# tatsy/opengl-raytracer

Measured on AMD Instinct MI355X. Metric: Mrays/s at 1920x1080, 8 bounces, higher is better.
Workload: dtype f32

## Files before the change

### opengl-raytracer_amd/csrc/glrtx.hip

```cpp
#include "glrtx.h"

#include <hip/hip_runtime.h>

#include <algorithm>
#include <cmath>
#include <cstdarg>
#include <cstdio>
#include <cstdlib>
#include <cstring>
#include <new>
#include <limits>
#include <string>
#include <vector>

#include "glrt_host.h"
#include "pt_kernel.hip.h"
#include "lbvh.hip.h"
#include "sahl.hip.h"
#include "refit.hip.h"
#include "query.hip.h"
#include "features.hip.h"
#include "denoise.hip.h"
#include "variance.hip.h"
#include "reproject.hip.h"
// ... 893 lines not shown
    P.ring = ring;
    P.inv_gamma = 1.0f / gamma;
    P.flip = flip ? 1 : 0;
    P.full = full;
    P.seq = P.acq = 0;
    P.timed = false;
    if (c->width > 0) {
        int rc = ensure(c, P.dev, present_image_bytes(c) * (size_t)ring);
        for (auto &im : P.img) {
            if (rc != GLRTX_OK || full) break;
            const hipError_t e = hipHostMalloc((void **)&im.host, std::max<size_t>(present_image_bytes(c), 64), hipHostMallocPortable);
            if (e != hipSuccess) rc = fail(c, GLRTX_ENOMEM, "glrtx_present_enable: pinned host memory: %s", hipGetErrorString(e));
            else im.host_bytes = std::max<size_t>(present_image_bytes(c), 64);
        }
        if (rc != GLRTX_OK) { (void)present_stop(c); return rc; }
    }
    return GLRTX_OK;
}

bool present_held(const glrtx_ctx *c) {
    for (const auto &im : c->pres.img)
        if (im.state == glrtx_ctx::Present::Image::HELD) return true;
    return false;
}

int wgwf_fetch(const glrtx_ctx *c, bool vine) {
    int fetch = vine ? 0 : ((size_t)c->n_fork + (size_t)c->st.n_tri >= (size_t)kPairFetchMinRecords ? 1 : 0);
    if (const char *v = std::getenv("GLRTX_PAIR_FETCH")) fetch = vine ? 0 : std::max(0, std::min(2, std::atoi(v)));
    return fetch;
}

int wgwf_lds_base(const glrtx_ctx *c) {
    return c->sc.lds_head_f4 * (int)sizeof(float4) + 2 * c->sc.stack_entries * kBlockThreads * (int)sizeof(int) + kWgCtlWords * (int)sizeof(unsigned) +
           2 * (int)sizeof(float4) + kCamFloatsPadded * (int)sizeof(float) + kLdsSeeds * (int)sizeof(float2) + kWgPathsMax / 8;
}

bool wgwf_compact(const glrtx_ctx *c, bool vine, int fetch) {
    const int lds_compact = wgwf_lds_base(c) + c->sc.n_crank * (int)sizeof(uint2);
    bool compact = !vine && fetch == 0 && c->sc.n_crank > 0 && (size_t)lds_compact * GLRTX_WGWF_WAVES <= (size_t)160 * 1024;
    if (const char *v = std::getenv("GLRTX_COMPACT_NODES")) compact = std::atoi(v) != 0 && !vine && fetch == 0 && c->sc.n_crank > 0 && lds_compact <= 160 * 1024;
    return compact;
}

int launch_wgwf(glrtx_ctx *c, const KernelArgs &a_in, const glrtx_params *p, const float *seeds_xy, int n_frames) {
    KernelArgs a = a_in;
    const int tiles8_x = (c->width + 7) / 8, tiles8_y = (c->owned_rows + 7) / 8;
    const size_t total = (size_t)tiles8_x * tiles8_y * 64;
    if (total * 2 >= (size_t)INT32_MAX) return fail(c, GLRTX_EINVAL, "image too large for the wgwf variant");
    const size_t plane_bytes = (size_t)a.pitch_f4 * (size_t)c->owned_rows * sizeof(float4);
    const size_t frame_bytes = (size_t)std::max(p->n_samples, 1) * plane_bytes;
    int rc;
    const bool busy = c->last_render_done && hipEventQuery(c->last_render_done) == hipErrorNotReady;
    (void)hipGetLastError();
    const bool burst = c->last_was_render && busy && same_camera(c->last_p, *p);
    const bool adapt = c->adapt_launch;
    const bool vol = c->ext_flags != 0;
    const bool moments = c->moments_launch;
    bool fed = !adapt && !moments && c->feed_ok && std::getenv("GLRTX_NO_FEED") == nullptr && c->pipeline && c->stream == c->own_stream && p->n_samples >= 1 && seeds_xy != nullptr && (n_frames > 1 || burst);
    int fed_cap = fed ? std::min(frames_cap(c, p, (int)kFedSlots), kFeedMaxFrames) : 0;
    if (const char *v = std::getenv("GLRTX_FEED_CAP")) fed_cap = std::max(1, std::min(fed_cap, std::atoi(v)));
    if (fed && n_frames > fed_cap) fed = false;
    bool piped = fed || (!adapt && !moments && n_frames == 1 && c->pipeline && p->n_samples >= 1 && (size_t)p->n_samples * plane_bytes <= ((size_t)1 << 30));
    const size_t ids = total * (size_t)(fed ? fed_cap : n_frames);
    if (ids + 1 >= (size_t)UINT32_MAX)
        return fail(c, GLRTX_EINVAL, "glrtx_render_frames: %d frames of %zu pixels exceed the 32-bit ray id space", n_frames, total);

    using Kernel = void (*)(const KernelArgs, const WfArgs, unsigned *, float4 *, const int *, const unsigned *, const VolArgs);
// ... 128 lines not shown
    w.tiles8_x = tiles8_x;
    w.refill_min = kRefillMin;
    if (const char *v = std::getenv("GLRTX_REFILL_MIN")) w.refill_min = std::max(1, std::min(64, std::atoi(v)));
    w.n_frames = fed ? std::max(fed_cap, 2) : n_frames;
    w.tiles_per_frame = (int)(total >> 6);
    const size_t plane_f4 = (size_t)a.pitch_f4 * (size_t)c->owned_rows;
    const int n_planes = n_frames * p->n_samples;
    if (fed) {
        FeedHost *fh = slot->feed_h;
        for (int i = 0; i < n_frames; i++) fh->seeds[i] = make_float2(seeds_xy[2 * i], seeds_xy[2 * i + 1]);
        __atomic_store_n(&fh->frames_pub, (unsigned)n_frames, __ATOMIC_RELEASE);
        w.feed_host = slot->feed_h_dev;
        w.feed_dev = (FeedDev *)slot->feed_d.p;
        w.feed_plane_f4 = plane_f4;
        w.feed_margin = 64 * 4 * grid;
        if (const char *v = std::getenv("GLRTX_FEED_MARGIN")) w.feed_margin = std::max(0, std::atoi(v));
    } else {
        if (n_frames > 1) {
            if ((rc = ensure(c, c->wfSeeds, (size_t)n_frames * sizeof(float2)))) return rc;
            HIP_TRY(c, hipMemcpyAsync(c->wfSeeds.p, seeds_xy, (size_t)n_frames * sizeof(float2), hipMemcpyHostToDevice, c->stream));
            w.seeds = (const float2 *)c->wfSeeds.p;
            w.seeds_in_lds = n_frames <= kLdsSeeds ? 1 : 0;
        }
        if (n_frames > 1 || slot || adapt || moments) {
            if ((rc = ensure(c, planeBuf, (size_t)std::max(n_planes, 1) * plane_f4 * sizeof(float4)))) return rc;
            w.planes = (float4 *)planeBuf.p;
        }
    }
    w.block_paths = block_paths;
    w.gss_div = (slot && !fed) ? 0 : 4 * grid;
    if (const char *v = std::getenv("GLRTX_GSS_DIV")) w.gss_div = std::max(0, std::atoi(v));
    w.suspend_max = kSuspendMax;
    if (const char *v = std::getenv("GLRTX_SUSPEND_MAX")) w.suspend_max = std::max(0, std::min(64, std::atoi(v)));
    w.trip_limit = (int)std::min<long long>(INT32_MAX, 64ll * std::max(p->n_samples, 1) * (p->max_depth + 2) + 64);
    if (vol) w.trip_limit = (int)std::min<long long>(INT32_MAX, 64ll * std::max(p->n_samples, 1) * 9 * (p->max_depth + 2) + 64);
    if (const char *v = std::getenv("GLRTX_TRIP_LIMIT")) w.trip_limit = std::max(1, std::atoi(v));
    w.err = c->guard_dev;
    {
        const size_t max_id = ids - 1;
        const size_t max_sidx = (size_t)kWfSetPlanes * state_entries + (size_t)grid * block_paths - 1;
        const size_t slice_f4 = 2 * (size_t)2 * 2 * block_paths  + (2 * (size_t)block_paths * sizeof(unsigned) + 15) / 16 ;
        static_assert(kWgSuspendAt + (size_t)kSuspendF4 * kBlockThreads == kWgQueueF4, "the suspend area closes a workgroup's slice");
        bool ok = slice_f4 <= kWgSuspendAt && max_id < (size_t)WF_INVALID && 2 * max_sidx + 1 < (size_t)WF_INVALID && (size_t)grid * block_paths <= state_entries &&
                  (size_t)kWfStatePlanes * state_entries * sizeof(float4) < ((size_t)1 << 32) && (block_paths & (block_paths - 1)) == 0 && block_paths >= 256 &&
                  block_paths <= kWgPathsMax && slice_f4 <= kWgQueueF4 && queueBuf.bytes >= (size_t)grid * kWgQueueF4 * sizeof(float4) &&
                  stateBuf.bytes >= state_bytes && w.ids == state_entries && grid >= 1 && (size_t)grid <= wg_slots &&
                  p->max_depth <= kWfDepthMax && p->n_samples <= kWfSampleMax && workPtr != nullptr;
        if (vol) ok = ok && p->n_samples <= kWfVolSampleMax && c->ext_flags == GLRTX_EXT_VOLUME && c->have_volume && c->vol.density != nullptr &&
                      c->vol.temperature != nullptr && c->n_spheres == 0 && !vine && fetch == 0 && !compact;
        if (!fed && n_frames > 1) ok = ok && c->wfSeeds.bytes >= (size_t)n_frames * sizeof(float2);
        if (w.planes) ok = ok && planeBuf.bytes >= (size_t)std::max(n_planes, 1) * plane_f4 * sizeof(float4);
        if (adapt) ok = ok && !fed && !slot && w.planes && c->ad_selected && c->ad_tiles == (int)(total >> 6) && c->adList.bytes >= (total >> 6) * sizeof(int) &&
                      c->adMask.bytes >= (total >> 6) && c->adHalf.bytes >= (size_t)c->ad_pitch * c->owned_rows && c->ad_pitch == c->pitch_bytes;
        if (moments) ok = ok && !fed && !slot && w.planes && c->mmM.p && c->mm_pitch == c->pitch_bytes && c->mm_rows == c->owned_rows &&
                        c->mmM.bytes >= c->pitch_bytes * (size_t)c->owned_rows;
        if (fed) ok = ok && n_frames >= 1 && n_frames <= fed_cap && fed_cap <= kFeedMaxFrames && slot->feed_d.bytes >= sizeof(FeedDev) && w.feed_host != nullptr &&
                      slot->chunks[(n_frames - 1) / kFeedChunkFrames].p != nullptr && slot->chunk_bytes == frame_bytes;
        if (!ok) return fail(c, GLRTX_EDEVICE, "internal: wgwf launch shapes inconsistent (ids %zu, max id %zu, grid %d of %zu slots (%d per CU), block_paths %d, frames %d, fed %d)", ids, max_id,
                             grid, wg_slots, per_cu, block_paths, n_frames, (int)fed);
        (void)queue_bytes_max;
    }
    glrtx_ctx::LaunchRec *rec = nullptr;
    if ((rc = next_launch_rec(c, rec))) return rc;
    if (slot && slot->used) HIP_TRY(c, hipStreamWaitEvent(rstream, slot->acc_done, 0));
    if (ctx_state && c->state_used) HIP_TRY(c, hipStreamWaitEvent(rstream, c->state_done, 0));
    HIP_TRY(c, hipMemsetAsync(workPtr, 0, sizeof(unsigned), rstream));
// ... 2680 lines not shown
```

### opengl-raytracer_amd/csrc/pt_kernel.hip.h

```cpp
#pragma once
#include <hip/hip_runtime.h>
#include <stdint.h>

#include "trav_asm.hip.h"
#include "scan_asm.hip.h"

namespace glrtx {

constexpr int kBlockThreads = 256;
constexpr int kTile = 16;
constexpr int REF_ABSENT = INT32_MIN;
constexpr int REF_FIN = INT32_MIN;
constexpr int kMaxLdsMaterials = 256;
constexpr int kMaxLdsLights = 64;
constexpr int kTopForks = 128;

constexpr float PT_EPS = 1.0e-4f;
constexpr float PT_INFTY = 1.0e8f;
constexpr float PT_PI = 3.14159274101257324f;
constexpr float PT_2PI = 6.28318548202514648f;

struct DevScene {
    const float4 *forks;
    const float4 *nodes0;
// ... 1406 lines not shown
struct FeedDev {
    unsigned frames_known;
    unsigned pad[31];
    unsigned long long seeds[kFeedMaxFrames];
    unsigned long long chunks[kFeedChunks];
};
constexpr int kCamFloatsPadded = 36;
constexpr int kLdsSeeds = 64;
constexpr int kWfSetPlanes = 6;
struct WfArgs {
    float4 *state;
    size_t ids;
    DEV size_t plane(int k) const { size_t n = ids; asm volatile("" : "+s"(n)); return (size_t)k * n; }
    DEV float4 *A(int k, unsigned sidx) const { return reinterpret_cast<float4 *>(reinterpret_cast<char *>(state + plane(k)) + (size_t)(sidx * 16u)); }
    DEV float4 *H(unsigned sidx) const { return A(5, sidx); }
    DEV unsigned set_base(int set, int wg) const { size_t n = ids; asm volatile("" : "+s"(n)); return (unsigned)((size_t)set * kWfSetPlanes * n) + (unsigned)wg * (unsigned)block_paths; }
    int total;
    int tiles8_x;
    int refill_min;
    int block_paths;
    int gss_div;
    int suspend_max;
    int trip_limit;
    unsigned *err;
    FeedHost *feed_host;
    FeedDev *feed_dev;
    size_t feed_plane_f4;
    int feed_margin;
    const float2 *seeds;
    int seeds_in_lds;
    float4 *planes;
    int n_frames;
    int tiles_per_frame;
    DEV void split(int id, int &frame, int &pid) const {
        if (n_frames > 1) { frame = (int)((unsigned)id / (unsigned)total); pid = id - frame * total; }
        else { frame = 0; pid = id; }
    }
};
constexpr int kWfStatePlanes = 2 * kWfSetPlanes;
constexpr int kWfDepthMax = 255;
constexpr int kWfSampleMax = (1 << 20) - 1;
constexpr int kWfVolSampleMax = (1 << 16) - 1;
constexpr unsigned kWfVolShift = 24;
constexpr unsigned kWfVolPassed = 9;
constexpr unsigned WF_PENDING = 1u << 28;
constexpr unsigned WF_FINISHING = 1u << 29;
constexpr unsigned WF_RESOLVED = 1u << 30;
constexpr unsigned WF_ACCEPTED = 1u << 31;
constexpr unsigned WF_INVALID = 0xFFFFFFFFu;
constexpr int kSuspendMax = 24;
constexpr float kHitSuspended = -1.0f;
constexpr int kSuspendF4 = 4;
constexpr int kRefillMin = 16;
#ifdef GLRTX_FAULT_INJECT
constexpr unsigned kFaultPoison = 0xFFFFFFFEu;
#endif

DEV bool wf_pixel(const KernelArgs &a, const WfArgs &w, int id, int &lx, int &lrow) {
    int frame, pid;
    w.split(id, frame, pid);
    const int t = pid >> 6, k = pid & 63;
    lx = (t % w.tiles8_x) * 8 + (k & 7);
    lrow = (t / w.tiles8_x) * 8 + (k >> 3);
    return lx < a.width && lrow < a.owned_rows;
}

// ... 219 lines not shown
    }
    if (ended) {
        int lx, lrow;
        wf_pixel(a, w, (int)id, lx, lrow);
        const int gy = local_row_to_y(a, lrow);
        const float fcx = (float)lx + 0.5f, fcy = (float)gy + 0.5f;
        wf_add_sample(a, w, (int)id, lx, lrow, sample, P.Lx, P.Ly, P.Lz);
        sample++;
        push_ext = wf_start(a, w, cam, (int)id, lx, lrow, rng, fcx, fcy, P, sample);
        if (push_ext) {
            ray_o = make_float4(P.ox, P.oy, P.oz, rng.x);
            ray_d = make_float4(P.dx, P.dy, P.dz, rng.y);
            st2 = make_float4(1.f, 1.f, 1.f, __uint_as_float(sample << 8));
            st3 = make_float4(0.f, 0.f, 0.f, s3.w);
        }
    } else {
        push_sh = sh.has_shadow;
        push_ext = !sh.ended;
        const unsigned m2 = (unsigned)P.depth | (sample << 8) | (push_sh ? WF_PENDING : 0u) | (sh.ended ? WF_FINISHING : 0u);
        ray_o = make_float4(P.ox, P.oy, P.oz, rng.x);
        ray_d = make_float4(P.dx, P.dy, P.dz, rng.y);
        st2 = make_float4(P.bx, P.by, P.bz, __uint_as_float(m2));
        st3 = make_float4(sh.Lpx, sh.Lpy, sh.Lpz, s3.w);
        if (push_sh) { st4 = make_float4(sh.Lfx, sh.Lfy, sh.Lfz, 0.f); has4 = true; }
        ray_sd = make_float4(sh.sdx, sh.sdy, sh.sdz, sh.dist);
    }
}

#ifndef GLRTX_STEPS_PER_TRIP
#define GLRTX_STEPS_PER_TRIP 6
#endif
constexpr int kWgCtlWords = 32;
constexpr int kWgPathsMax = 4096;
constexpr size_t kWgSuspendAt = 8 * (size_t)kWgPathsMax + (size_t)kWgPathsMax / 2;
constexpr size_t kWgQueueF4 = kWgSuspendAt + (size_t)kSuspendF4 * kBlockThreads;
#ifndef GLRTX_PRIO_TRAVERSE
#define GLRTX_PRIO_TRAVERSE 3
#define GLRTX_PRIO_SHADE 0
#endif
#ifndef GLRTX_WGWF_WAVES
#define GLRTX_WGWF_WAVES 4
#endif

#ifdef GLRTX_PHASE_STATS
__device__ unsigned long long g_phase_cycles[8];
__device__ uint4 g_trip_log[16][64];
#define PH_STAMP(var) const unsigned long long var = __builtin_amdgcn_s_memtime()
#define PH_ADD(i, t0, t1) do { if (threadIdx.x == 0) atomicAdd(&g_phase_cycles[i], (t1) - (t0)); } while (0)
#else
#define PH_STAMP(var)
#define PH_ADD(i, t0, t1)
#endif

#ifdef GLRTX_RAY_LOG
struct RayLog { float4 *rays; uint2 *trips; unsigned long long cap_rays; unsigned cap_trips; unsigned on; };
__device__ RayLog g_ray_log;
__device__ unsigned long long g_ray_log_n;
__device__ unsigned g_ray_log_trips;
#endif

DEV int wgwf_suspend_max();

template <bool VINE, int FETCH>
DEV void wg_traverse_phase(const KernelArgs &a, const WfArgs &w, const float4 *root, int *stack, const float4 *rq, int n_rays,
                           unsigned *ray_head, unsigned *light_bits, unsigned long long &rays, float4 *suspend_area) {
    const int lane = threadIdx.x & 63;
    const uint2 *ranks = reinterpret_cast<const uint2 *>(light_bits + kWgPathsMax / 32);
    if (VINE) {
        for (;;) {
            int base = 0;
            if (lane == 0) base = (int)atomicAdd(ray_head, 64u);
            base = __builtin_amdgcn_readfirstlane(base);
            if (base >= n_rays) break;
            float4 o = make_float4(0.f, 0.f, 0.f, __uint_as_float(WF_INVALID)), d = o;
            if (base + lane < n_rays) { o = ld_stream(&rq[2 * (size_t)(base + lane)]); d = ld_stream(&rq[2 * (size_t)(base + lane) + 1]); }
            const unsigned r = __float_as_uint(o.w);
            const bool shadow = (r & 1u) != 0u;
            const Hit h = trav_scan<true>(a.sc, o.x, o.y, o.z, d.x, d.y, d.z, r != WF_INVALID, shadow ? shadow_limit(d.w, a.sc.shadow_limited) : PT_INFTY,
                                          shadow ? d.w : -__builtin_inff());
            if (r != WF_INVALID) {
                rays++;
                if (r & 1u) { if (nee_accepted(d.w, h.t, h.tri >= 0)) atomicOr(&light_bits[r >> 6], 1u << ((r >> 1) & 31u)); }
                else st_stream(w.H(r >> 1), make_float4(h.t, __int_as_float(h.tri), h.u, h.v));
            }
        }
        return;
    }
    const unsigned long long lt_mask = (1ull << lane) - 1ull;
    const float4 none = make_float4(0.f, 0.f, 0.f, __uint_as_float(WF_INVALID));
    float4 cur_o = none, cur_d = none;
    float cur_ix = 0.f, cur_iy = 0.f, cur_iz = 0.f;
    int cur_pos = 0, cur_cnt = 0;
    auto fetch = [&](float4 &o, float4 &d) -> int {
        int base = 0;
        if (lane == 0) base = (int)atomicAdd(ray_head, 64u);
        base = __builtin_amdgcn_readfirstlane(base);
        int cnt = n_rays - base;
        cnt = cnt < 0 ? 0 : (cnt > 64 ? 64 : cnt);
        if (lane < cnt) {
            o = ld_stream(&rq[2 * (size_t)(base + lane)]);
// ... 12 lines not shown
    bool active = false;
    bool unsaved = false;
    unsigned rid = 0;
    Trav T;
    T.cur = 0; T.sp = 0;
    T.h.t = PT_INFTY; T.h.tri = -1; T.h.u = 0.f; T.h.v = 0.f;
#ifdef GLRTX_STEP_TIMING
    StepTiming step_timing;
#endif
    float4 *const susp = suspend_area + (size_t)kSuspendF4 * threadIdx.x;
    {
        const float4 s3 = susp[3];
        if (s3.z != 0.0f) {
            const float4 s0 = susp[0], s1 = susp[1], s2 = susp[2];
            susp[3] = make_float4(0.f, 0.f, 0.f, 0.f);
            T.ox = s0.x; T.oy = s0.y; T.oz = s0.z;
            rid = __float_as_uint(w.H(__float_as_uint(s0.w) >> 1)->y);
#ifdef GLRTX_FAULT_INJECT
            const bool fault_dropped = rid == kFaultPoison;
#endif
            T.dx = s1.x; T.dy = s1.y; T.dz = s1.z; T.stop_d = s1.w;
            T.ix = frcp(T.dx); T.iy = frcp(T.dy); T.iz = frcp(T.dz);
            T.h.t = s2.x; T.h.tri = __float_as_int(s2.y); T.h.u = s2.z; T.h.v = s2.w;
            T.cur = __float_as_int(s3.x); T.sp = __float_as_int(s3.y);
#ifdef GLRTX_TRAV_STATS
            T.iters = 0;
#endif
            active = true;
#ifdef GLRTX_FAULT_INJECT
            if (fault_dropped) active = false;
#endif
        }
    }
    auto save_hit = [&]() {
        const unsigned id = rid >> 1;
        if (rid & 1u) {
            if (nee_accepted(T.stop_d, T.h.t, T.h.tri >= 0)) atomicOr(&light_bits[id >> 5], 1u << (id & 31u));
        } else *w.H(id) = make_float4(T.h.t, __int_as_float(T.h.tri), T.h.u, T.h.v);
        unsaved = false;
    };
#ifdef GLRTX_PHASE_STATS
    unsigned long long ph_refill = 0ull, ph_refills = 0ull, ph_step = 0ull;
#endif
    for (;;) {
        unsigned long long idle = __ballot(!active);
        if ((int)__popcll(idle) >= w.refill_min || idle == ~0ull) {
#ifdef GLRTX_PHASE_STATS
            const unsigned long long rf0 = __builtin_amdgcn_s_memtime();
#endif
            while (idle != 0ull && !exhausted) {
                if (cur_pos >= cur_cnt) {
                    cur_cnt = cur_cnt == 64 ? fetch(cur_o, cur_d) : 0;
                    cur_pos = 0;
                    if (cur_cnt == 0) { exhausted = true; break; }
                }
                const int n = __popcll(idle);
                const int avail = cur_cnt - cur_pos;
                const int take = n < avail ? n : avail;
                const int rank = __popcll(idle & lt_mask);
                const int src = (cur_pos + rank) & 63;
                const float ox = __shfl(cur_o.x, src), oy = __shfl(cur_o.y, src), oz = __shfl(cur_o.z, src);
                const unsigned new_rid = (unsigned)__shfl((int)__float_as_uint(cur_o.w), src);
                const float dx = __shfl(cur_d.x, src), dy = __shfl(cur_d.y, src), dz = __shfl(cur_d.z, src);
                const float dist_m = __shfl(cur_d.w, src);
                const float ix = __shfl(cur_ix, src), iy = __shfl(cur_iy, src), iz = __shfl(cur_iz, src);
                if (!active && rank < take) {
                    if (unsaved) save_hit();
                    rid = new_rid;
                    if (rid != WF_INVALID) {
                        rays++;
                        const bool shadow = (rid & 1u) != 0u;
                        const float dist = __builtin_fabsf(dist_m);
                        T.ox = ox; T.oy = oy; T.oz = oz; T.dx = dx; T.dy = dy; T.dz = dz; T.ix = ix; T.iy = iy; T.iz = iz;
                        T.h.t = shadow ? shadow_limit(dist, a.sc.shadow_limited) : PT_INFTY; T.h.tri = -1; T.h.u = 0.f; T.h.v = 0.f;
                        T.stop_d = shadow ? dist : -__builtin_inff();
                        T.sp = 0;
                        T.cur = (FETCH & kWgwfCompact) ? 0 : a.sc.root_ref;
#ifdef GLRTX_TRAV_STATS
                        T.iters = 0;
#endif
                        active = (__float_as_uint(dist_m) & 0x80000000u) == 0u;
                        unsaved = !active;
                    }
                }
                cur_pos += take;
                idle = __ballot(!active);
            }
#ifdef GLRTX_PHASE_STATS
            ph_refill += __builtin_amdgcn_s_memtime() - rf0; ph_refills += 1ull;
#endif
        }
        if (!__any(active)) {
            if (exhausted) break;
            continue;
        }
        if (exhausted && fetched_any) {
            const unsigned long long ma = __ballot(active);
            const int suspend_max = wgwf_suspend_max();
            if (__ballot(active && (rid & 1u) != 0u) == 0ull && (int)__popcll(ma) <= suspend_max) {
                if (active) {
                    susp[0] = make_float4(T.ox, T.oy, T.oz, __uint_as_float(rid));
                    susp[1] = make_float4(T.dx, T.dy, T.dz, T.stop_d);
                    susp[2] = make_float4(T.h.t, __int_as_float(T.h.tri), T.h.u, T.h.v);
                    susp[3] = make_float4(__int_as_float(T.cur), __int_as_float(T.sp), 1.0f, 0.f);
                    float mark = kHitSuspended, zero = 0.f;
                    asm volatile("" : "+v"(mark), "+v"(zero));
                    *w.H(rid >> 1) = make_float4(mark, zero, zero, zero);
                    active = false;
                }
                break;
            }
        }
#ifdef GLRTX_PHASE_STATS
        const unsigned long long sb0 = __builtin_amdgcn_s_memtime();
#endif
#ifdef GLRTX_TRAV_STATS
        {
            const unsigned long long ma = __ballot(active);
            if (lane == 0) {
                atomicAdd(&g_trav_trips[0], 1ull); atomicAdd(&g_trav_trips[1], (unsigned long long)__popcll(ma));
                if (exhausted) { atomicAdd(&g_trav_trips[2], 1ull); atomicAdd(&g_trav_trips[3], (unsigned long long)__popcll(ma)); }
            }
        }
#endif
        if (active) {
#if defined(GLRTX_TRAV_STATS) || defined(GLRTX_CXX_STEP)
            constexpr bool CP = (FETCH & kWgwfCompact) != 0;
            bool fin = trav_step<true, CP>(a.sc, stack, T, ranks);
#pragma unroll
            for (int k = 1; k < GLRTX_STEPS_PER_TRIP; k++)
                if (!fin) fin = trav_step<true, CP>(a.sc, stack, T, ranks);
#else
#ifdef GLRTX_STEP_TIMING
            trav_steps_asm<FETCH>(a.sc, stack, T, (unsigned)(uintptr_t)ranks, step_timing);
#else
            trav_steps_asm<FETCH>(a.sc, stack, T, (unsigned)(uintptr_t)ranks);
#endif
            const bool fin = T.cur == REF_FIN;
#endif
            if (fin) {
                active = false;
                unsaved = true;
            }
        }
#ifdef GLRTX_PHASE_STATS
        ph_step += __builtin_amdgcn_s_memtime() - sb0;
#endif
    }
    if (unsaved) save_hit();
#ifdef GLRTX_PHASE_STATS
    if (threadIdx.x == 0) { atomicAdd(&g_phase_cycles[5], ph_refill); atomicAdd(&g_phase_cycles[6], ph_refills); atomicAdd(&g_phase_cycles[7], ph_step); }
#endif
#ifdef GLRTX_STEP_TIMING
    atomicAdd(&g_step_timing[0], (unsigned long long)step_timing.n);
    atomicAdd(&g_step_timing[1], (unsigned long long)step_timing.t);
    atomicAdd(&g_step_timing[2], (unsigned long long)step_timing.w);
#endif
}

template <bool VOL = false>
DEV void wg_shade_phase(const KernelArgs &a, const WfArgs &w, const float4 *lds_mats, const float *cam, const unsigned *light_bits, int n_paths,
                        float4 *rq_next, unsigned *n_rays_next, unsigned *n_paths_next, unsigned cur_base, unsigned next_base, unsigned long long &rays,
                        unsigned *moved) {
    const int lane = threadIdx.x & 63;
    const unsigned long long lt_mask = (1ull << lane) - 1ull;
    for (int j0 = 0; j0 < n_paths; j0 += kBlockThreads) {
        const int i = j0 + (int)threadIdx.x;
        bool push_ext = false, push_sh = false, requeue = false, has4 = false;
        unsigned id = WF_INVALID;
        float4 ro = make_float4(0.f, 0.f, 0.f, 0.f), rd = ro, rsd = ro, st2 = ro, st3 = ro, st4 = ro;
        const bool light_accepted = i < n_paths && ((light_bits[i >> 5] >> (i & 31)) & 1u) != 0u;
        if (i < n_paths)
            wf_shade_path<VOL>(a, w, lds_mats, cam, id, cur_base + (unsigned)i, light_accepted, push_ext, push_sh, requeue, ro, rd, rsd, st2, st3, st4, has4, rays);
        const unsigned long long me = __ballot(push_ext), ms = __ballot(push_sh), mq = __ballot(requeue), mp = me | ms | mq;
        const unsigned long long mv = __ballot(id != WF_INVALID);
        unsigned br = 0, bp = 0;
        if (lane == 0) {
            if (mv & ~mq) *moved = 1u;
            if (mp) {
                br = atomicAdd(n_rays_next, (unsigned)(__popcll(me) + __popcll(ms)));
                bp = atomicAdd(n_paths_next, (unsigned)__popcll(mp));
            }
        }
        br = __builtin_amdgcn_readfirstlane(br);
        bp = __builtin_amdgcn_readfirstlane(bp);
        const unsigned pos_next = bp + (unsigned)__popcll(mp & lt_mask);
        const unsigned sidx_next = next_base + pos_next;
        if (push_ext || push_sh || requeue) {
            st_stream(w.A(0, sidx_next), ro);
            st_stream(w.A(1, sidx_next), rd);
            st_stream(w.A(2, sidx_next), st2);
            st_stream(w.A(3, sidx_next), st3);
            if (has4) st_stream(w.A(4, sidx_next), st4);
        }
#ifdef GLRTX_FAULT_INJECT
        if (requeue) {
            *w.H(cur_base + (unsigned)i) = make_float4(kHitSuspended, __uint_as_float(kFaultPoison), 0.f, 0.f);
            *w.H(sidx_next) = make_float4(kHitSuspended, 0.f, 0.f, 0.f);
        }
#else
        if (requeue) *w.H(cur_base + (unsigned)i) = make_float4(kHitSuspended, __uint_as_float(sidx_next * 2u), 0.f, 0.f);
#endif
        if (push_ext) {
            float4 *r = rq_next + 2 * (size_t)(br + __popcll(me & lt_mask));
            r[0] = make_float4(ro.x, ro.y, ro.z, __uint_as_float(sidx_next * 2u));
            r[1] = make_float4(rd.x, rd.y, rd.z, 0.f);
        }
        if (push_sh) {
            float4 *r = rq_next + 2 * (size_t)(br + __popcll(me) + __popcll(ms & lt_mask));
            r[0] = make_float4(ro.x, ro.y, ro.z, __uint_as_float(pos_next * 2u + 1u));
            r[1] = rsd;
        }
    }
}

struct WgwfKernArgs {
    KernelArgs a;
    WfArgs w;
    unsigned *work_counter;
    float4 *wg_queues;
    const int *adapt_list;
    const unsigned *adapt_count;
    VolArgs vol;
};
DEV const WgwfKernArgs *wgwf_kernargs() {
    auto p = __builtin_amdgcn_kernarg_segment_ptr();
    asm volatile("" : "+s"(p));
    return (const WgwfKernArgs *)p;
}

DEV int wgwf_suspend_max() { return wgwf_kernargs()->w.suspend_max; }
DEV const VolArgs *wgwf_vol() { return &wgwf_kernargs()->vol; }

template <bool VOL = false>
DEV void wg_feed_topup(int kWgPaths, unsigned *ctl, int cur, unsigned *work_counter) {
    const WgwfKernArgs *k = wgwf_kernargs();
    FeedHost *fh = k->w.feed_host;
    FeedDev *fd = k->w.feed_dev;
    int lane = threadIdx.x;
    if constexpr (VOL) asm volatile("" : "+v"(lane));
    const int tpf = k->w.tiles_per_frame, gss_div = k->w.gss_div;
    const int np = (int)ctl[4 + cur];
    const bool may_take = ctl[7] == 0u && ctl[13] == 0u;
    int want = (kWgPaths - np) >> 6;
    unsigned kw = __hip_atomic_load(&fd->frames_known, __ATOMIC_RELAXED, __HIP_MEMORY_SCOPE_AGENT);
    int known = (int)(kw & ~kFeedClosed);
    bool closed = (kw & kFeedClosed) != 0u;
    const int done = (int)__hip_atomic_load(work_counter, __ATOMIC_RELAXED, __HIP_MEMORY_SCOPE_AGENT);
    unsigned wg_id = blockIdx.x;
    asm volatile("" : "+s"(wg_id));
    const bool looker = (wg_id & 31u) == 0u || np == 0;
    if (looker && may_take && want > 0 && !closed && known * tpf - done < k->w.feed_margin) {
        unsigned v = 0u;
        if (lane == 0) v = __hip_atomic_load(&fh->frames_pub, __ATOMIC_RELAXED, __HIP_MEMORY_SCOPE_SYSTEM);
        v = (unsigned)__builtin_amdgcn_readfirstlane((int)v);
        int pub = (int)(v & ~kFeedClosed);
        pub = pub > kFeedMaxFrames ? kFeedMaxFrames : pub;
        if (pub > known) {
            for (int f = known + lane; f < pub; f += 64) {
                const float sx = __hip_atomic_load(&fh->seeds[f].x, __ATOMIC_RELAXED, __HIP_MEMORY_SCOPE_SYSTEM), sy = __hip_atomic_load(&fh->seeds[f].y, __ATOMIC_RELAXED, __HIP_MEMORY_SCOPE_SYSTEM);
                __hip_atomic_store(&fd->seeds[f], (unsigned long long)__float_as_uint(sx) | ((unsigned long long)__float_as_uint(sy) << 32), __ATOMIC_RELAXED, __HIP_MEMORY_SCOPE_AGENT);
            }
            for (int c = known / kFeedChunkFrames + lane; c <= (pub - 1) / kFeedChunkFrames; c += 64) {
                unsigned long long ptr = __hip_atomic_load(reinterpret_cast<unsigned long long *>(&fh->chunks[c]), __ATOMIC_RELAXED, __HIP_MEMORY_SCOPE_SYSTEM);
                __hip_atomic_store(&fd->chunks[c], ptr, __ATOMIC_RELAXED, __HIP_MEMORY_SCOPE_AGENT);
// ... 21 lines not shown
    }
    int base = 0, got = 0;
    unsigned p_lo = ctl[16], p_hi = ctl[17];
    if (may_take) {
        if (p_lo < p_hi) {
            const int v_hi = (int)p_hi < n_tiles ? (int)p_hi : n_tiles;
            if ((int)p_lo < v_hi) { base = (int)p_lo; got = v_hi - (int)p_lo; p_lo += (unsigned)got; }
        } else if (want > 0 && !closed) {
            base = (int)atomicAdd(work_counter, (unsigned)want);
            const int hi = base + want;
            const int v_hi = hi < n_tiles ? hi : (base < n_tiles ? n_tiles : base);
            got = v_hi - base;
            if (hi > v_hi) { p_lo = (unsigned)v_hi; p_hi = (unsigned)hi; }
        }
    }
    unsigned again = 0u;
    if (may_take && got == 0 && np == 0) {
        if (!closed) {
            unsigned expect = (unsigned)known;
            if (__hip_atomic_compare_exchange_strong(&fh->frames_pub, &expect, (unsigned)known | kFeedClosed, __ATOMIC_RELAXED, __ATOMIC_RELAXED, __HIP_MEMORY_SCOPE_SYSTEM) ||
                expect == ((unsigned)known | kFeedClosed)) {
                __hip_atomic_fetch_max(&fd->frames_known, (unsigned)known | kFeedClosed, __ATOMIC_RELAXED, __HIP_MEMORY_SCOPE_AGENT);
                closed = true;
            } else again = 1u;
        }
    }
    const unsigned turns = again ? ctl[15] + 1u : 0u;
    ctl[15] = turns;
    if (turns > 4096u) {
        unsigned *e = k->w.err;
        __hip_atomic_store(e + 1, (unsigned)known, __ATOMIC_RELAXED, __HIP_MEMORY_SCOPE_SYSTEM);
        __hip_atomic_store(e + 2, turns, __ATOMIC_RELAXED, __HIP_MEMORY_SCOPE_SYSTEM);
        __hip_atomic_store(e + 3, 0u, __ATOMIC_RELAXED, __HIP_MEMORY_SCOPE_SYSTEM);
        __hip_atomic_store(e, 3u, __ATOMIC_RELAXED, __HIP_MEMORY_SCOPE_SYSTEM);
        ctl[13] = 1u;
        again = 0u;
    }
    if (closed && (int)p_lo >= n_tiles) { ctl[7] = 1u; p_lo = p_hi = 0u; }
    ctl[16] = p_lo; ctl[17] = p_hi;
    ctl[0] = (unsigned)base; ctl[6] = (unsigned)got; ctl[14] = again;
    if (np > 0) ctl[12] = got > 0 ? 0u : ctl[12] + 1u;
}

constexpr int kWgwfAdaptive = 4;
template <bool COUNT_RAYS, bool VINE, int FETCH = 0>
__global__ __launch_bounds__(kBlockThreads, GLRTX_WGWF_WAVES) void pt_render_wgwf(const KernelArgs a, const WfArgs w, unsigned *work_counter, float4 *wg_queues,
                                                                                  const int * , const unsigned * , const VolArgs ) {
    constexpr bool ADAPT = (FETCH & kWgwfAdaptive) != 0;
    constexpr bool VOL = (FETCH & kWgwfVolume) != 0;
    constexpr int NODE_FETCH = FETCH & ~(kWgwfAdaptive | kWgwfVolume);
    static_assert(!VOL || (!VINE && NODE_FETCH == 0), "the V form has the one-record-per-lane fetch on DevScene::nodes only");
    extern __shared__ __attribute__((aligned(16))) unsigned char lds_raw[];
    float4 *lds_mats = reinterpret_cast<float4 *>(lds_raw);
    const int mat_f4 = a.sc.lds_head_f4;
    unsigned char *pl = lds_raw + (size_t)mat_f4 * sizeof(float4);
    int *stack = reinterpret_cast<int *>(pl) + 2 * threadIdx.x;
    pl += (size_t)2 * a.sc.stack_entries * kBlockThreads * sizeof(int);
    unsigned *ctl = reinterpret_cast<unsigned *>(pl);
    float4 *lds_root = reinterpret_cast<float4 *>(pl + kWgCtlWords * sizeof(unsigned));
    float *lds_cam = reinterpret_cast<float *>(pl + kWgCtlWords * sizeof(unsigned) + 32);
    unsigned *light_bits = reinterpret_cast<unsigned *>(pl + kWgCtlWords * sizeof(unsigned) + 32 + kCamFloatsPadded * 4 + kLdsSeeds * 8);
    if (threadIdx.x < kCamFloats) lds_cam[threadIdx.x] = a.cam[threadIdx.x];
    if (w.seeds_in_lds && (int)threadIdx.x < 2 * w.n_frames) lds_cam[kCamFloatsPadded + threadIdx.x] = reinterpret_cast<const float *>(w.seeds)[threadIdx.x];
    if (threadIdx.x == 64) lds_root[0] = a.sc.root_lo;
    if (threadIdx.x == 65) lds_root[1] = a.sc.root_hi;
    float4 *rayQ = wg_queues + (size_t)blockIdx.x * kWgQueueF4;
    if (a.sc.mats_in_lds) stage_mats(a, lds_mats);
    stage_lights(a, lds_mats);
    if (FETCH & kWgwfCompact) {
        uint2 *lds_ranks = reinterpret_cast<uint2 *>(light_bits + kWgPathsMax / 32);
        for (int i = threadIdx.x; i < a.sc.n_crank; i += kBlockThreads) lds_ranks[i] = a.sc.cranks[i];
    }

    const int kWgPaths = w.block_paths;
    unsigned long long rays = 0;
#ifdef GLRTX_PHASE_STATS
    if (threadIdx.x == 0 && (blockIdx.x & 63) == 0 && blockIdx.x / 64 < 16)
        g_trip_log[blockIdx.x / 64][0].y = (unsigned)(__builtin_amdgcn_s_memtime() >> 4);
#endif
    if (threadIdx.x == 0) { ctl[2] = 0u; ctl[3] = 0u; ctl[4] = 0u; ctl[5] = 0u; ctl[7] = 0u; ctl[10] = 0u; ctl[11] = 0u; ctl[12] = 0u; ctl[13] = 0u; ctl[14] = 0u; ctl[15] = 0u; ctl[16] = 0u; ctl[17] = 0u; ctl[18] = 0u; }
    if (!VINE) rayQ[kWgSuspendAt + (size_t)kSuspendF4 * threadIdx.x + 3] = make_float4(0.f, 0.f, 0.f, 0.f);
    int cur = 0;
    __syncthreads();
    for (;;) {
        PH_STAMP(pg0);
        unsigned tid_topup = threadIdx.x;
        asm volatile("" : "+v"(tid_topup));
        if (wgwf_kernargs()->w.feed_dev != nullptr) {
            if (tid_topup < 64u) wg_feed_topup<VOL>(kWgPaths, ctl, cur, work_counter);
        } else if (tid_topup == 0u) {
            const int n_tiles = (ADAPT ? (int)*wgwf_kernargs()->adapt_count : wgwf_kernargs()->w.tiles_per_frame) * wgwf_kernargs()->w.n_frames;
            int want = (kWgPaths - (int)ctl[4 + cur]) >> 6;
            int base = 0, got = 0;
            const int gss_div = wgwf_kernargs()->w.gss_div;
            if (want > 0 && ctl[7] == 0u && gss_div > 0) {
                const int left = n_tiles - (int)__hip_atomic_load(work_counter, __ATOMIC_RELAXED, __HIP_MEMORY_SCOPE_AGENT);
                const int share = left > 0 ? (left + gss_div - 1) / gss_div : 1;
                want = want < share ? want : share;
            }
            if (want > 0 && ctl[7] == 0u && ctl[13] == 0u) {
                base = (int)atomicAdd(work_counter, (unsigned)want);
                got = base < n_tiles ? (want < n_tiles - base ? want : n_tiles - base) : 0;
                if (base + want >= n_tiles) ctl[7] = 1u;
            }
            ctl[0] = (unsigned)base; ctl[6] = (unsigned)got; ctl[14] = 0u;
            ctl[12] = got > 0 ? 0u : ctl[12] + 1u;
        }
        __syncthreads();
        if (ctl[13] != 0u) break;
        const bool look_again = ctl[14] != 0u;
        {
            const int got = (int)ctl[6] * 64, tile0 = (int)ctl[0];
            {
                unsigned tid = threadIdx.x;
                asm volatile("" : "+v"(tid));
                if (tid < kWgPathsMax / 32) light_bits[tid] = 0u;
            }
            const int nr = (int)ctl[2 + cur], np = (int)ctl[4 + cur];
            float4 *rq_w = rayQ + 2 * ((size_t)cur * 2 * kWgPaths + nr);
            const WgwfKernArgs *kt = wgwf_kernargs();
            const unsigned new_base = kt->w.set_base(cur, (int)blockIdx.x) + (unsigned)np;
            for (int k = threadIdx.x; k < got; k += kBlockThreads) {
                int id = tile0 * 64 + k;
                if (ADAPT) {
                    const int g = tile0 + (k >> 6), n_active = (int)*kt->adapt_count;
                    const int frame = g / n_active;
                    id = frame * kt->w.total + kt->adapt_list[g - frame * n_active] * 64 + (k & 63);
                }
                float4 ro = make_float4(0.f, 0.f, 0.f, __uint_as_float(WF_INVALID)), rd = ro;
                const bool go = wf_generate_one(kt->a, kt->w, lds_cam, id, new_base + (unsigned)k, ro, rd);
                rq_w[2 * k] = ro;
                rq_w[2 * k + 1] = rd;
                (void)go;
            }
            __syncthreads();
            if (tid_topup == 0u) { ctl[2 + cur] = (unsigned)(nr + got); ctl[4 + cur] = (unsigned)(np + got); ctl[1] = 0u; }
        }
        __syncthreads();
        PH_STAMP(pg1);
        PH_ADD(0, pg0, pg1);
        const int n_rays = (int)ctl[2 + cur], n_paths = (int)ctl[4 + cur];
        if (n_paths == 0) {
            if (look_again) continue;
            break;
        }
        const float4 *rq = rayQ + 2 * ((size_t)cur * 2 * kWgPaths);

#ifdef GLRTX_RAY_LOG
        if (g_ray_log.on) {
            if (threadIdx.x == 0) {
                const unsigned long long base = atomicAdd(&g_ray_log_n, (unsigned long long)n_rays);
                ctl[9] = 0u;
                if (base + (unsigned long long)n_rays <= g_ray_log.cap_rays) {
                    const unsigned t = atomicAdd(&g_ray_log_trips, 1u);
                    if (t < g_ray_log.cap_trips) { g_ray_log.trips[t] = make_uint2((unsigned)base, (unsigned)n_rays); ctl[8] = (unsigned)base; ctl[9] = 1u; }
                }
            }
            __syncthreads();
            if (ctl[9]) {
                float4 *dst = g_ray_log.rays + 2 * (size_t)ctl[8];
                for (int i = threadIdx.x; i < 2 * n_rays; i += kBlockThreads) dst[i] = rq[i];
            }
            __syncthreads();
        }
#endif
        PH_STAMP(pt0);
        __builtin_amdgcn_s_setprio(GLRTX_PRIO_TRAVERSE);
        wg_traverse_phase<VINE, NODE_FETCH>(a, w, lds_root, stack, rq, n_rays, &ctl[1], light_bits, rays, rayQ + kWgSuspendAt);
        __builtin_amdgcn_s_setprio(GLRTX_PRIO_SHADE);
        PH_STAMP(pt1);
        __syncthreads();
        PH_STAMP(pt2);
        PH_ADD(1, pt0, pt1);
        PH_ADD(2, pt1, pt2);

        const WgwfKernArgs *ks = wgwf_kernargs();
        wg_shade_phase<VOL>(ks->a, ks->w, lds_mats, lds_cam, light_bits, n_paths, rayQ + 2 * ((size_t)(cur ^ 1) * 2 * kWgPaths),
                            &ctl[2 + (cur ^ 1)], &ctl[4 + (cur ^ 1)], ks->w.set_base(cur, (int)blockIdx.x), ks->w.set_base(cur ^ 1, (int)blockIdx.x), rays, &ctl[10]);
        PH_STAMP(ps1);
        __syncthreads();
        PH_STAMP(ps2);
        PH_ADD(3, pt2, ps1);
        PH_ADD(4, ps1, ps2);
#ifdef GLRTX_PHASE_STATS
        if (threadIdx.x == 0 && (blockIdx.x & 63) == 0 && blockIdx.x / 64 < 16) {
            uint4 *lg = g_trip_log[blockIdx.x / 64];
            const unsigned n = lg[0].x + 1u;
            if (n < 64u) { lg[n] = make_uint4((unsigned)n_rays, (unsigned)n_paths, (unsigned)(pt2 - pt0), (unsigned)(ps2 - pt2)); lg[0].x = n; }
        }
#endif
        unsigned tid_end = threadIdx.x;
        asm volatile("" : "+v"(tid_end));
        if (tid_end == 0u) {
            ctl[2 + cur] = 0u; ctl[4 + cur] = 0u;
            const bool idle = n_rays == 0 && ctl[10] == 0u;
            ctl[10] = 0u;
            const unsigned idle_trips = idle ? ctl[11] + 1u : 0u;
            ctl[11] = idle_trips;
            const WgwfKernArgs *kg = wgwf_kernargs();
            const unsigned code = idle_trips >= 2u ? 1u : (ctl[12] > (unsigned)kg->w.trip_limit ? 2u : 0u);
            if (code != 0u) {
                unsigned *e = kg->w.err;
                unsigned wg;
                asm volatile("v_mov_b32 %0, %1" : "=v"(wg) : "s"((unsigned)blockIdx.x));
                __hip_atomic_store(e + 1, wg, __ATOMIC_RELAXED, __HIP_MEMORY_SCOPE_SYSTEM);
                __hip_atomic_store(e + 2, ctl[12], __ATOMIC_RELAXED, __HIP_MEMORY_SCOPE_SYSTEM);
                __hip_atomic_store(e + 3, ctl[4 + (cur ^ 1)], __ATOMIC_RELAXED, __HIP_MEMORY_SCOPE_SYSTEM);
                __hip_atomic_store(e, code, __ATOMIC_RELEASE, __HIP_MEMORY_SCOPE_SYSTEM);
                ctl[13] = 1u;
            }
        }
        cur ^= 1;
    }
#ifdef GLRTX_PHASE_STATS
    if (threadIdx.x == 0 && (blockIdx.x & 63) == 0 && blockIdx.x / 64 < 16)
        g_trip_log[blockIdx.x / 64][0].z = (unsigned)(__builtin_amdgcn_s_memtime() >> 4);
#endif
    flush_rays<COUNT_RAYS>(a, rays);
}

#ifdef GLRTX_RAY_LOG
template <int FETCH>
__global__ __launch_bounds__(kBlockThreads, GLRTX_WGWF_WAVES) void pt_replay_traverse(const KernelArgs a, const WfArgs w, unsigned *work_counter, float4 *wg_queues,
                                                                                      const float4 *log, const uint2 *trips, int n_trips) {
    extern __shared__ __attribute__((aligned(16))) unsigned char lds_raw[];
    const int mat_f4 = a.sc.lds_head_f4;
    unsigned char *pl = lds_raw + (size_t)mat_f4 * sizeof(float4);
    int *stack = reinterpret_cast<int *>(pl) + 2 * threadIdx.x;
    pl += (size_t)2 * a.sc.stack_entries * kBlockThreads * sizeof(int);
    unsigned *ctl = reinterpret_cast<unsigned *>(pl);
    float4 *lds_root = reinterpret_cast<float4 *>(pl + kWgCtlWords * sizeof(unsigned));
    unsigned *light_bits = reinterpret_cast<unsigned *>(pl + kWgCtlWords * sizeof(unsigned) + 32 + kCamFloatsPadded * 4 + kLdsSeeds * 8);
    if (threadIdx.x == 64) lds_root[0] = a.sc.root_lo;
    if (threadIdx.x == 65) lds_root[1] = a.sc.root_hi;
    float4 *rayQ = wg_queues + (size_t)blockIdx.x * kWgQueueF4;
    rayQ[kWgSuspendAt + (size_t)kSuspendF4 * threadIdx.x + 3] = make_float4(0.f, 0.f, 0.f, 0.f);
    unsigned long long rays = 0;
    __syncthreads();
    for (;;) {
        if (threadIdx.x == 0) { ctl[0] = atomicAdd(work_counter, 1u); ctl[1] = 0u; }
        if (threadIdx.x < kWgPathsMax / 32) light_bits[threadIdx.x] = 0u;
        __syncthreads();
        const unsigned t = ctl[0];
        if (t >= (unsigned)n_trips) break;
        const uint2 tr = trips[t];
        __builtin_amdgcn_s_setprio(GLRTX_PRIO_TRAVERSE);
        wg_traverse_phase<false, FETCH>(a, w, lds_root, stack, log + 2 * (size_t)tr.x, (int)tr.y, &ctl[1], light_bits, rays, rayQ + kWgSuspendAt);
        __builtin_amdgcn_s_setprio(GLRTX_PRIO_SHADE);
        __syncthreads();
    }
    flush_rays<true>(a, rays);
}
#endif

__global__ __launch_bounds__(256) void accumulate_planes_kernel(float4 *accum, int pitch_f4, int width, int rows, const float4 *planes,
                                                                int n_planes) {
    const int x = blockIdx.x * 64 + (threadIdx.x & 63);
    const int y = blockIdx.y * 4 + (threadIdx.x >> 6);
    if (x >= width || y >= rows) return;
    const size_t at = (size_t)y * pitch_f4 + x, plane = (size_t)rows * pitch_f4;
    float4 acc = accum[at];
    for (int k = 0; k < n_planes; k++) {
        const float4 v = planes[(size_t)k * plane + at];
        acc.x = acc.x + v.x; acc.y = acc.y + v.y; acc.z = acc.z + v.z;
        acc.w = acc.w + 1.0f;
    }
    accum[at] = acc;
}

__global__ __launch_bounds__(64) void feed_prefill_kernel(FeedDev *fd, const FeedHost *fh, int n_frames) {
    const int lane = threadIdx.x;
    for (int f = lane; f < n_frames; f += 64) fd->seeds[f] = (unsigned long long)__float_as_uint(fh->seeds[f].x) | ((unsigned long long)__float_as_uint(fh->seeds[f].y) << 32);
    for (int c = lane; c <= (n_frames - 1) / kFeedChunkFrames; c += 64) fd->chunks[c] = (unsigned long long)fh->chunks[c];
    if (lane == 0) fd->frames_known = (unsigned)n_frames;
}

__global__ __launch_bounds__(256) void accumulate_feed_kernel(float4 *accum, int pitch_f4, int width, int rows, const FeedDev *fd, int n_samples) {
    const int x = blockIdx.x * 64 + (threadIdx.x & 63);
    const int y = blockIdx.y * 4 + (threadIdx.x >> 6);
    if (x >= width || y >= rows) return;
// ... 232 lines not shown
```

Before: 10330.

## Let shade phase start per 64-path group before traversal fully finishes

Adds per-group completion counters in LDS so that waves claim 64-path shading groups dynamically and, when enabled, wait only for that group's rays to finish rather than for a workgroup-wide barrier after traversal. Traversal increments group counters as hits are saved, and shading or generation records how many rays each next-phase group needs. The early mode is gated by an environment variable and off by default, but the default path still picks up the dynamic group claiming and extra LDS atomics. It also closes the feed on abort.

```diff
diff --git a/opengl-raytracer_amd/csrc/glrtx.hip b/opengl-raytracer_amd/csrc/glrtx.hip
--- a/opengl-raytracer_amd/csrc/glrtx.hip
+++ b/opengl-raytracer_amd/csrc/glrtx.hip
@@ -949,7 +949,7 @@
 
 int wgwf_lds_base(const glrtx_ctx *c) {
     return c->sc.lds_head_f4 * (int)sizeof(float4) + 2 * c->sc.stack_entries * kBlockThreads * (int)sizeof(int) + kWgCtlWords * (int)sizeof(unsigned) +
-           2 * (int)sizeof(float4) + kCamFloatsPadded * (int)sizeof(float) + kLdsSeeds * (int)sizeof(float2) + kWgPathsMax / 8;
+           2 * (int)sizeof(float4) + kCamFloatsPadded * (int)sizeof(float) + kLdsSeeds * (int)sizeof(float2) + kWgPathsMax / 8 + kWgGroupWords * (int)sizeof(unsigned);
 }
 
 bool wgwf_compact(const glrtx_ctx *c, bool vine, int fetch) {
@@ -1144,6 +1144,8 @@
     if (const char *v = std::getenv("GLRTX_GSS_DIV")) w.gss_div = std::max(0, std::atoi(v));
     w.suspend_max = kSuspendMax;
     if (const char *v = std::getenv("GLRTX_SUSPEND_MAX")) w.suspend_max = std::max(0, std::min(64, std::atoi(v)));
+    w.shade_early = 0;
+    if (const char *v = std::getenv("GLRTX_SHADE_EARLY")) w.shade_early = std::atoi(v) != 0 ? 1 : 0;
     w.trip_limit = (int)std::min<long long>(INT32_MAX, 64ll * std::max(p->n_samples, 1) * (p->max_depth + 2) + 64);
     if (vol) w.trip_limit = (int)std::min<long long>(INT32_MAX, 64ll * std::max(p->n_samples, 1) * 9 * (p->max_depth + 2) + 64);
     if (const char *v = std::getenv("GLRTX_TRIP_LIMIT")) w.trip_limit = std::max(1, std::atoi(v));
diff --git a/opengl-raytracer_amd/csrc/pt_kernel.hip.h b/opengl-raytracer_amd/csrc/pt_kernel.hip.h
--- a/opengl-raytracer_amd/csrc/pt_kernel.hip.h
+++ b/opengl-raytracer_amd/csrc/pt_kernel.hip.h
@@ -1462,6 +1462,7 @@
     float4 *planes;
     int n_frames;
     int tiles_per_frame;
+    int shade_early;
     DEV void split(int id, int &frame, int &pid) const {
         if (n_frames > 1) { frame = (int)((unsigned)id / (unsigned)total); pid = id - frame * total; }
         else { frame = 0; pid = id; }
@@ -1747,6 +1748,10 @@
 #endif
 constexpr int kWgCtlWords = 32;
 constexpr int kWgPathsMax = 4096;
+constexpr int kWgGroups = kWgPathsMax / 64;
+constexpr int kWgLightWords = kWgPathsMax / 32;
+constexpr int kWgGroupWords = 2 * kWgGroups;
+constexpr unsigned kGroupDone = 0x10000u;
 constexpr size_t kWgSuspendAt = 8 * (size_t)kWgPathsMax + (size_t)kWgPathsMax / 2;
 constexpr size_t kWgQueueF4 = kWgSuspendAt + (size_t)kSuspendF4 * kBlockThreads;
 #ifndef GLRTX_PRIO_TRAVERSE
@@ -1775,12 +1780,13 @@
 #endif
 
 DEV int wgwf_suspend_max();
+DEV int wgwf_block_paths();
 
 template <bool VINE, int FETCH>
 DEV void wg_traverse_phase(const KernelArgs &a, const WfArgs &w, const float4 *root, int *stack, const float4 *rq, int n_rays,
-                           unsigned *ray_head, unsigned *light_bits, unsigned long long &rays, float4 *suspend_area) {
+                           unsigned *ray_head, unsigned *light_bits, unsigned long long &rays, float4 *suspend_area, unsigned *grp) {
     const int lane = threadIdx.x & 63;
-    const uint2 *ranks = reinterpret_cast<const uint2 *>(light_bits + kWgPathsMax / 32);
+    const uint2 *ranks = reinterpret_cast<const uint2 *>(light_bits + kWgLightWords + kWgGroupWords);
     if (VINE) {
         for (;;) {
             int base = 0;
@@ -1859,11 +1865,27 @@
 #endif
         }
     }
+    unsigned owed = 0u;
+    auto group_of = [&](unsigned r) -> unsigned {
+        return ((r & 1u) ? r >> 7 : ((r >> 1) & (unsigned)(wgwf_block_paths() - 1)) >> 6) & (unsigned)(kWgGroups - 1);
+    };
+    auto pay = [&]() {
+        if (owed != 0u) {
+            __hip_atomic_fetch_add(&grp[owed - 1u], kGroupDone, __ATOMIC_RELEASE, __HIP_MEMORY_SCOPE_WORKGROUP);
+            owed = 0u;
+        }
+    };
     auto save_hit = [&]() {
         const unsigned id = rid >> 1;
         if (rid & 1u) {
             if (nee_accepted(T.stop_d, T.h.t, T.h.tri >= 0)) atomicOr(&light_bits[id >> 5], 1u << (id & 31u));
-        } else *w.H(id) = make_float4(T.h.t, __int_as_float(T.h.tri), T.h.u, T.h.v);
+            asm volatile("" ::: "memory");
+            __hip_atomic_fetch_add(&grp[group_of(rid)], kGroupDone, __ATOMIC_RELAXED, __HIP_MEMORY_SCOPE_WORKGROUP);
+        } else {
+            *w.H(id) = make_float4(T.h.t, __int_as_float(T.h.tri), T.h.u, T.h.v);
+            pay();
+            owed = 1u + group_of(rid);
+        }
         unsaved = false;
     };
 #ifdef GLRTX_PHASE_STATS
@@ -1875,6 +1897,7 @@
 #ifdef GLRTX_PHASE_STATS
             const unsigned long long rf0 = __builtin_amdgcn_s_memtime();
 #endif
+            pay();
             while (idle != 0ull && !exhausted) {
                 if (cur_pos >= cur_cnt) {
                     cur_cnt = cur_cnt == 64 ? fetch(cur_o, cur_d) : 0;
@@ -1926,6 +1949,8 @@
             const int suspend_max = wgwf_suspend_max();
             if (__ballot(active && (rid & 1u) != 0u) == 0ull && (int)__popcll(ma) <= suspend_max) {
                 if (active) {
+                    pay();
+                    owed = 1u + group_of(rid);
                     susp[0] = make_float4(T.ox, T.oy, T.oz, __uint_as_float(rid));
                     susp[1] = make_float4(T.dx, T.dy, T.dz, T.stop_d);
                     susp[2] = make_float4(T.h.t, __int_as_float(T.h.tri), T.h.u, T.h.v);
@@ -1975,6 +2000,7 @@
 #endif
     }
     if (unsaved) save_hit();
+    pay();
 #ifdef GLRTX_PHASE_STATS
     if (threadIdx.x == 0) { atomicAdd(&g_phase_cycles[5], ph_refill); atomicAdd(&g_phase_cycles[6], ph_refills); atomicAdd(&g_phase_cycles[7], ph_step); }
 #endif
@@ -1985,14 +2011,45 @@
 #endif
 }
 
+DEV void wg_group_need(unsigned *grp, unsigned pos_first, unsigned pos, unsigned long long m_a, unsigned long long m_b, unsigned long long m_c) {
+    const unsigned g0 = pos_first >> 6;
+    const unsigned long long m0 = __ballot((pos >> 6) == g0);
+    const unsigned c0 = (unsigned)(__popcll(m_a & m0) + __popcll(m_b & m0) + __popcll(m_c & m0));
+    const unsigned c1 = (unsigned)(__popcll(m_a & ~m0) + __popcll(m_b & ~m0) + __popcll(m_c & ~m0));
+    if ((threadIdx.x & 63) == 0) {
+        if (c0 != 0u) atomicAdd(&grp[g0], c0);
+        if (c1 != 0u) atomicAdd(&grp[g0 + 1u], c1);
+    }
+}
+
 template <bool VOL = false>
 DEV void wg_shade_phase(const KernelArgs &a, const WfArgs &w, const float4 *lds_mats, const float *cam, const unsigned *light_bits, int n_paths,
                         float4 *rq_next, unsigned *n_rays_next, unsigned *n_paths_next, unsigned cur_base, unsigned next_base, unsigned long long &rays,
-                        unsigned *moved) {
+                        unsigned *moved, bool early, unsigned *claim, unsigned *arrived, unsigned *grp_cur, unsigned *grp_next) {
     const int lane = threadIdx.x & 63;
     const unsigned long long lt_mask = (1ull << lane) - 1ull;
-    for (int j0 = 0; j0 < n_paths; j0 += kBlockThreads) {
-        const int i = j0 + (int)threadIdx.x;
+    const int n_groups = (n_paths + 63) >> 6;
+    for (;;) {
+        int g = 0;
+        if (lane == 0) g = (int)atomicAdd(claim, 1u);
+        g = __builtin_amdgcn_readfirstlane(g);
+        if (g >= n_groups) break;
+        if (early) {
+#ifdef GLRTX_PHASE_STATS
+            const unsigned long long sw0 = __builtin_amdgcn_s_memtime();
+#endif
+            for (;;) {
+                const unsigned v = (unsigned)__builtin_amdgcn_readfirstlane((int)__hip_atomic_load(&grp_cur[g], __ATOMIC_ACQUIRE, __HIP_MEMORY_SCOPE_WORKGROUP));
+                if ((v & 0xFFFFu) == (v >> 16)) break;
+                const unsigned n = (unsigned)__builtin_amdgcn_readfirstlane((int)__hip_atomic_load(arrived, __ATOMIC_ACQUIRE, __HIP_MEMORY_SCOPE_WORKGROUP));
+                if (n >= (unsigned)(kBlockThreads / 64)) break;
+                __builtin_amdgcn_s_sleep(4);
+            }
+#ifdef GLRTX_PHASE_STATS
+            if (threadIdx.x == 0) atomicAdd(&g_phase_cycles[2], __builtin_amdgcn_s_memtime() - sw0);
+#endif
+        }
+        const int i = g * 64 + lane;
         bool push_ext = false, push_sh = false, requeue = false, has4 = false;
         unsigned id = WF_INVALID;
         float4 ro = make_float4(0.f, 0.f, 0.f, 0.f), rd = ro, rsd = ro, st2 = ro, st3 = ro, st4 = ro;
@@ -2013,6 +2070,7 @@
         bp = __builtin_amdgcn_readfirstlane(bp);
         const unsigned pos_next = bp + (unsigned)__popcll(mp & lt_mask);
         const unsigned sidx_next = next_base + pos_next;
+        wg_group_need(grp_next, bp, pos_next, me, ms, mq);
         if (push_ext || push_sh || requeue) {
             st_stream(w.A(0, sidx_next), ro);
             st_stream(w.A(1, sidx_next), rd);
@@ -2057,7 +2115,15 @@
 }
 
 DEV int wgwf_suspend_max() { return wgwf_kernargs()->w.suspend_max; }
+DEV int wgwf_block_paths() { return wgwf_kernargs()->w.block_paths; }
 DEV const VolArgs *wgwf_vol() { return &wgwf_kernargs()->vol; }
+
+DEV void wg_feed_close_on_abort() {
+    const WgwfKernArgs *k = wgwf_kernargs();
+    if (k->w.feed_dev == nullptr) return;
+    __hip_atomic_fetch_or(&k->w.feed_host->frames_pub, kFeedClosed, __ATOMIC_RELAXED, __HIP_MEMORY_SCOPE_SYSTEM);
+    __hip_atomic_fetch_or(&k->w.feed_dev->frames_known, kFeedClosed, __ATOMIC_RELAXED, __HIP_MEMORY_SCOPE_AGENT);
+}
 
 template <bool VOL = false>
 DEV void wg_feed_topup(int kWgPaths, unsigned *ctl, int cur, unsigned *work_counter) {
@@ -2145,7 +2211,8 @@
         __hip_atomic_store(e + 1, (unsigned)known, __ATOMIC_RELAXED, __HIP_MEMORY_SCOPE_SYSTEM);
         __hip_atomic_store(e + 2, turns, __ATOMIC_RELAXED, __HIP_MEMORY_SCOPE_SYSTEM);
         __hip_atomic_store(e + 3, 0u, __ATOMIC_RELAXED, __HIP_MEMORY_SCOPE_SYSTEM);
-        __hip_atomic_store(e, 3u, __ATOMIC_RELAXED, __HIP_MEMORY_SCOPE_SYSTEM);
+        __hip_atomic_store(e, 3u, __ATOMIC_RELEASE, __HIP_MEMORY_SCOPE_SYSTEM);
+        wg_feed_close_on_abort();
         ctl[13] = 1u;
         again = 0u;
     }
@@ -2180,8 +2247,10 @@
     float4 *rayQ = wg_queues + (size_t)blockIdx.x * kWgQueueF4;
     if (a.sc.mats_in_lds) stage_mats(a, lds_mats);
     stage_lights(a, lds_mats);
+    unsigned *grp = light_bits + kWgLightWords;
+    if (threadIdx.x < kWgGroupWords) grp[threadIdx.x] = 0u;
     if (FETCH & kWgwfCompact) {
-        uint2 *lds_ranks = reinterpret_cast<uint2 *>(light_bits + kWgPathsMax / 32);
+        uint2 *lds_ranks = reinterpret_cast<uint2 *>(light_bits + kWgLightWords + kWgGroupWords);
         for (int i = threadIdx.x; i < a.sc.n_crank; i += kBlockThreads) lds_ranks[i] = a.sc.cranks[i];
     }
 
@@ -2191,7 +2260,7 @@
     if (threadIdx.x == 0 && (blockIdx.x & 63) == 0 && blockIdx.x / 64 < 16)
         g_trip_log[blockIdx.x / 64][0].y = (unsigned)(__builtin_amdgcn_s_memtime() >> 4);
 #endif
-    if (threadIdx.x == 0) { ctl[2] = 0u; ctl[3] = 0u; ctl[4] = 0u; ctl[5] = 0u; ctl[7] = 0u; ctl[10] = 0u; ctl[11] = 0u; ctl[12] = 0u; ctl[13] = 0u; ctl[14] = 0u; ctl[15] = 0u; ctl[16] = 0u; ctl[17] = 0u; ctl[18] = 0u; }
+    if (threadIdx.x == 0) { ctl[2] = 0u; ctl[3] = 0u; ctl[4] = 0u; ctl[5] = 0u; ctl[7] = 0u; ctl[10] = 0u; ctl[11] = 0u; ctl[12] = 0u; ctl[13] = 0u; ctl[14] = 0u; ctl[15] = 0u; ctl[16] = 0u; ctl[17] = 0u; ctl[18] = 0u; ctl[19] = 0u; ctl[20] = 0u; }
     if (!VINE) rayQ[kWgSuspendAt + (size_t)kSuspendF4 * threadIdx.x + 3] = make_float4(0.f, 0.f, 0.f, 0.f);
     int cur = 0;
     __syncthreads();
@@ -2227,7 +2296,8 @@
             {
                 unsigned tid = threadIdx.x;
                 asm volatile("" : "+v"(tid));
-                if (tid < kWgPathsMax / 32) light_bits[tid] = 0u;
+                if (tid < kWgLightWords) light_bits[tid] = 0u;
+                else if (tid < kWgLightWords + kWgGroups) grp[(cur ^ 1) * kWgGroups + (int)tid - kWgLightWords] = 0u;
             }
             const int nr = (int)ctl[2 + cur], np = (int)ctl[4 + cur];
             float4 *rq_w = rayQ + 2 * ((size_t)cur * 2 * kWgPaths + nr);
@@ -2244,10 +2314,10 @@
                 const bool go = wf_generate_one(kt->a, kt->w, lds_cam, id, new_base + (unsigned)k, ro, rd);
                 rq_w[2 * k] = ro;
                 rq_w[2 * k + 1] = rd;
-                (void)go;
+                wg_group_need(grp + cur * kWgGroups, (unsigned)(np + k - (int)(threadIdx.x & 63)), (unsigned)(np + k), __ballot(go), 0ull, 0ull);
             }
             __syncthreads();
-            if (tid_topup == 0u) { ctl[2 + cur] = (unsigned)(nr + got); ctl[4 + cur] = (unsigned)(np + got); ctl[1] = 0u; }
+            if (tid_topup == 0u) { ctl[2 + cur] = (unsigned)(nr + got); ctl[4 + cur] = (unsigned)(np + got); ctl[1] = 0u; ctl[19] = 0u; ctl[20] = 0u; }
         }
         __syncthreads();
         PH_STAMP(pg1);
@@ -2279,17 +2349,22 @@
 #endif
         PH_STAMP(pt0);
         __builtin_amdgcn_s_setprio(GLRTX_PRIO_TRAVERSE);
-        wg_traverse_phase<VINE, NODE_FETCH>(a, w, lds_root, stack, rq, n_rays, &ctl[1], light_bits, rays, rayQ + kWgSuspendAt);
+        wg_traverse_phase<VINE, NODE_FETCH>(a, w, lds_root, stack, rq, n_rays, &ctl[1], light_bits, rays, rayQ + kWgSuspendAt, grp + cur * kWgGroups);
         __builtin_amdgcn_s_setprio(GLRTX_PRIO_SHADE);
         PH_STAMP(pt1);
-        __syncthreads();
+        bool early = false;
+        if constexpr (!VINE && !VOL) early = wgwf_kernargs()->w.shade_early != 0;
+        if (early) {
+            if ((threadIdx.x & 63) == 0) __hip_atomic_fetch_add(&ctl[20], 1u, __ATOMIC_RELEASE, __HIP_MEMORY_SCOPE_WORKGROUP);
+        } else __syncthreads();
         PH_STAMP(pt2);
         PH_ADD(1, pt0, pt1);
         PH_ADD(2, pt1, pt2);
 
         const WgwfKernArgs *ks = wgwf_kernargs();
         wg_shade_phase<VOL>(ks->a, ks->w, lds_mats, lds_cam, light_bits, n_paths, rayQ + 2 * ((size_t)(cur ^ 1) * 2 * kWgPaths),
-                            &ctl[2 + (cur ^ 1)], &ctl[4 + (cur ^ 1)], ks->w.set_base(cur, (int)blockIdx.x), ks->w.set_base(cur ^ 1, (int)blockIdx.x), rays, &ctl[10]);
+                            &ctl[2 + (cur ^ 1)], &ctl[4 + (cur ^ 1)], ks->w.set_base(cur, (int)blockIdx.x), ks->w.set_base(cur ^ 1, (int)blockIdx.x), rays, &ctl[10],
+                            early, &ctl[19], &ctl[20], grp + cur * kWgGroups, grp + (cur ^ 1) * kWgGroups);
         PH_STAMP(ps1);
         __syncthreads();
         PH_STAMP(ps2);
@@ -2320,6 +2395,7 @@
                 __hip_atomic_store(e + 2, ctl[12], __ATOMIC_RELAXED, __HIP_MEMORY_SCOPE_SYSTEM);
                 __hip_atomic_store(e + 3, ctl[4 + (cur ^ 1)], __ATOMIC_RELAXED, __HIP_MEMORY_SCOPE_SYSTEM);
                 __hip_atomic_store(e, code, __ATOMIC_RELEASE, __HIP_MEMORY_SCOPE_SYSTEM);
+                wg_feed_close_on_abort();
                 ctl[13] = 1u;
             }
         }
@@ -2352,13 +2428,13 @@
     __syncthreads();
     for (;;) {
         if (threadIdx.x == 0) { ctl[0] = atomicAdd(work_counter, 1u); ctl[1] = 0u; }
-        if (threadIdx.x < kWgPathsMax / 32) light_bits[threadIdx.x] = 0u;
+        if (threadIdx.x < kWgLightWords + kWgGroupWords) light_bits[threadIdx.x] = 0u;
         __syncthreads();
         const unsigned t = ctl[0];
         if (t >= (unsigned)n_trips) break;
         const uint2 tr = trips[t];
         __builtin_amdgcn_s_setprio(GLRTX_PRIO_TRAVERSE);
-        wg_traverse_phase<false, FETCH>(a, w, lds_root, stack, log + 2 * (size_t)tr.x, (int)tr.y, &ctl[1], light_bits, rays, rayQ + kWgSuspendAt);
+        wg_traverse_phase<false, FETCH>(a, w, lds_root, stack, log + 2 * (size_t)tr.x, (int)tr.y, &ctl[1], light_bits, rays, rayQ + kWgSuspendAt, light_bits + kWgLightWords);
         __builtin_amdgcn_s_setprio(GLRTX_PRIO_SHADE);
         __syncthreads();
     }
```

Result: no change. 10260 (-0.7%).
